# voidful/DeSTA2.5-Audio

Hardware: AMD Instinct MI355X
Metric: train steps/sec (node) Whisper-v3+Llama3.1-8B Q-Former6L at 1/2/4/8 MI355X (higher is better)
Workload: dtype bf16

## Files before the change

desta2.5-audio_amd/csrc/gemm_bf16.hip:

```cpp
#include "common.h"
#include "desta_hip.h"
#include <math.h>

#ifndef GEMM_GROUP_M
#define GEMM_GROUP_M 8
#endif

namespace {

typedef __attribute__((ext_vector_type(4))) unsigned u32x4;
typedef __attribute__((ext_vector_type(2))) float f32x2;

constexpr int BM = 128, BN = 128, BK = 64;
constexpr int TILE_BYTES = BM * BK * 2;

struct GemmArgs {
    const bf16_t* A; const bf16_t* B; void* C;
    int M, N, K;
    long lda, ldb, ldc;
    long sA, sB, sC;
    const float* bias;
    const void* res; long ldr; long sR; int res_f32;
    int act;
    int out_f32;
    bf16_t* preact; long ldp; long sP;
    float alpha;
    bf16_t* aux; long lda_x;
    unsigned drop_thresh, seed_lo, seed_hi; float drop_scale;
    int tilesM, tilesN;
    int full_tiles, split;
    union {
        float* ws;
        const float* b_scale;
    };
    int* tickets;
    const float* rms_w; float rms_eps;
    const float* rope_cs; const int* rope_pos; int rope_cols, rope_hd;
    int tail_skip;
};

__device__ __forceinline__ void rope4(const GemmArgs& p, int m, int n0, float (&v)[4]) {
    if (p.rope_cs && n0 < p.rope_cols) {
        const int pos = p.rope_pos[m];
        const float4 cs = *(const float4*)(p.rope_cs + ((long)pos * (p.rope_hd >> 1) + ((n0 & (p.rope_hd - 1)) >> 1)) * 2);
        const float a0 = v[0], b0 = v[1], a1 = v[2], b1 = v[3];
        v[0] = a0 * cs.x - b0 * cs.y; v[1] = b0 * cs.x + a0 * cs.y;
        v[2] = a1 * cs.z - b1 * cs.w; v[3] = b1 * cs.z + a1 * cs.w;
    }
}

__device__ __forceinline__ void gelu4_bf16(float (&v)[4]) {
#pragma unroll
    for (int e = 0; e < 4; ++e) v[e] = gelu_erf_fast(v[e]);
}

__device__ __forceinline__ void glds16(const void* g, void* l) {
    __builtin_amdgcn_global_load_lds((const __attribute__((address_space(1))) void*)g,
                                     (__attribute__((address_space(3))) void*)l, 16, 0, 0);
}

template <bool ROPE = false>
__device__ __forceinline__ void epilogue4(const GemmArgs& p, int z, int m, int n0, const f32x4& a) {
    float v[4];
#pragma unroll
    for (int e = 0; e < 4; ++e) v[e] = a[e] * p.alpha;
    if (p.bias) {
        const float4 b = *(const float4*)(p.bias + n0);
        v[0] += b.x; v[1] += b.y; v[2] += b.z; v[3] += b.w;
    }
    if constexpr (ROPE) rope4(p, m, n0, v);
    if (p.preact) {
        u16x4 o;
#pragma unroll
        for (int e = 0; e < 4; ++e) o[e] = f2bf(v[e]);
        *(u16x4*)(p.preact + (long)z * p.sP + (long)m * p.ldp + n0) = o;
    }
    if (p.act == 1) {
        if (p.out_f32) {
#pragma unroll
            for (int e = 0; e < 4; ++e) v[e] = gelu_erf(v[e]);
        } else {
            gelu4_bf16(v);
        }
    }
    if (p.drop_thresh) {
        const unsigned long base = ((unsigned long)z * p.M + m) * p.N + n0;
#pragma unroll
        for (int e = 0; e < 4; ++e) v[e] = desta_keep(p.seed_lo, p.seed_hi, base + e, p.drop_thresh) ? v[e] * p.drop_scale : 0.f;
    }
    if (p.res) {
        if (p.res_f32) {
            const float4 r = *(const float4*)((const float*)p.res + (long)z * p.sR + (long)m * p.ldr + n0);
            v[0] += r.x; v[1] += r.y; v[2] += r.z; v[3] += r.w;
        } else {
            const u16x4 r = *(const u16x4*)((const bf16_t*)p.res + (long)z * p.sR + (long)m * p.ldr + n0);
#pragma unroll
            for (int e = 0; e < 4; ++e) v[e] += bf2f(r[e]);
        }
    }
    if (p.out_f32) {
        *(float4*)((float*)p.C + (long)z * p.sC + (long)m * p.ldc + n0) = make_float4(v[0], v[1], v[2], v[3]);
    } else {
        u16x4 o;
#pragma unroll
        for (int e = 0; e < 4; ++e) o[e] = f2bf(v[e]);
        *(u16x4*)((bf16_t*)p.C + (long)z * p.sC + (long)m * p.ldc + n0) = o;
    }
}

__device__ __forceinline__ void epilogue4_f32_stream(const GemmArgs& p, int z, int m, int n0, const f32x4& a) {
    const float4 b = *(const float4*)(p.bias + n0);
    const float4 r = *(const float4*)((const float*)p.res + (long)z * p.sR + (long)m * p.ldr + n0);
    *(float4*)((float*)p.C + (long)z * p.sC + (long)m * p.ldc + n0) =
        make_float4((a[0] * p.alpha + b.x) + r.x, (a[1] * p.alpha + b.y) + r.y, (a[2] * p.alpha + b.z) + r.z, (a[3] * p.alpha + b.w) + r.w);
}

template <int MODE = -1>
__device__ __forceinline__ void epilogue_pair_bf16(const GemmArgs& p, int z, int m, bool row_ok, int ncol0, int fq,
                                                   const f32x4& a0, const f32x4& a1) {
    constexpr bool DYN = MODE < 0;
    const bool has_bias = DYN ? p.bias != nullptr : (MODE & 1) != 0;
    const bool has_gelu = DYN ? p.act == 1 : (MODE & 2) != 0;
    const bool has_rope = DYN ? true : (MODE & 4) != 0;
    const bool has_res = DYN ? p.res != nullptr : (MODE & 8) != 0;
    const bool has_pre = DYN ? p.preact != nullptr : (MODE & 16) != 0;
    if (has_res && !p.res_f32 && (p.ldr & 7) == 0 && (p.sR & 7) == 0) {
        float v[2][4];
#pragma unroll
        for (int t = 0; t < 2; ++t) {
            const f32x4& a = t ? a1 : a0;
            const int n0 = ncol0 + t * 16 + fq * 4;
#pragma unroll
            for (int e = 0; e < 4; ++e) v[t][e] = a[e] * p.alpha;
            if (has_bias) {
                const float4 b = *(const float4*)(p.bias + n0);
                v[t][0] += b.x; v[t][1] += b.y; v[t][2] += b.z; v[t][3] += b.w;
            }
            if (has_gelu) gelu4_bf16(v[t]);
        }
        const int col = ncol0 + (fq & 1) * 16 + (fq >> 1) * 8;
        const u16x8 r = *(const u16x8*)((const bf16_t*)p.res + (long)z * p.sR + (long)m * p.ldr + col);
        float w[8];
#pragma unroll
        for (int e = 0; e < 4; ++e) {
            const auto sw = __builtin_amdgcn_permlane16_swap(__float_as_uint(v[0][e]), __float_as_uint(v[1][e]), false, false);
            w[e] = __uint_as_float(sw[0]);
            w[4 + e] = __uint_as_float(sw[1]);
        }
        u16x8 o;
#pragma unroll
        for (int e = 0; e < 8; ++e) o[e] = f2bf(w[e] + bf2f(r[e]));
        if (row_ok) *(u16x8*)((bf16_t*)p.C + (long)z * p.sC + (long)m * p.ldc + col) = o;
        return;
    }
    unsigned pk[2][2];
#pragma unroll
    for (int t = 0; t < 2; ++t) {
        const f32x4& a = t ? a1 : a0;
        const int n0 = ncol0 + t * 16 + fq * 4;
        float v[4];
#pragma unroll
        for (int e = 0; e < 4; ++e) v[e] = a[e] * p.alpha;
        if (has_bias) {
            const float4 b = *(const float4*)(p.bias + n0);
            v[0] += b.x; v[1] += b.y; v[2] += b.z; v[3] += b.w;
        }
        if (has_rope) rope4(p, min(m, p.M - 1), n0, v);
        if (has_gelu) gelu4_bf16(v);
        if (has_res) {
            if (p.res_f32) {
                const float4 r = *(const float4*)((const float*)p.res + (long)z * p.sR + (long)m * p.ldr + n0);
                v[0] += r.x; v[1] += r.y; v[2] += r.z; v[3] += r.w;
            } else {
                const u16x4 r = *(const u16x4*)((const bf16_t*)p.res + (long)z * p.sR + (long)m * p.ldr + n0);
#pragma unroll
                for (int e = 0; e < 4; ++e) v[e] += bf2f(r[e]);
            }
        }
        pk[t][0] = (unsigned)f2bf(v[0]) | ((unsigned)f2bf(v[1]) << 16);
        pk[t][1] = (unsigned)f2bf(v[2]) | ((unsigned)f2bf(v[3]) << 16);
    }
    const auto lo = __builtin_amdgcn_permlane16_swap(pk[0][0], pk[1][0], false, false);
    const auto hi = __builtin_amdgcn_permlane16_swap(pk[0][1], pk[1][1], false, false);
    const int col = ncol0 + (fq & 1) * 16 + (fq >> 1) * 8;
    if (row_ok) {
        const uint4 o = make_uint4(lo[0], hi[0], lo[1], hi[1]);
        *(uint4*)((bf16_t*)p.C + (long)z * p.sC + (long)m * p.ldc + col) = o;
        if (has_pre) *(uint4*)(p.preact + (long)z * p.sP + (long)m * p.ldp + col) = o;
    }
}

__device__ __forceinline__ uint4 pair_swap_pk(unsigned x0, unsigned x1, unsigned y0, unsigned y1) {
    const auto lo = __builtin_amdgcn_permlane16_swap(x0, y0, false, false);
    const auto hi = __builtin_amdgcn_permlane16_swap(x1, y1, false, false);
    return make_uint4(lo[0], hi[0], lo[1], hi[1]);
}
__device__ __forceinline__ unsigned pk2(float a, float b) { return (unsigned)f2bf(a) | ((unsigned)f2bf(b) << 16); }

__device__ __forceinline__ void epilogue_swiglu_fwd(const GemmArgs& p, int z, int m, bool row_ok, int ncol0, int fq,
                                                    const f32x4& a0, const f32x4& a1, const f32x4& a2, const f32x4& a3) {
    float g[2][4], u[2][4], o[2][4];
#pragma unroll
    for (int e = 0; e < 4; ++e) {
        g[0][e] = bf2f(f2bf(a0[e] * p.alpha)); g[1][e] = bf2f(f2bf(a1[e] * p.alpha));
        u[0][e] = bf2f(f2bf(a2[e] * p.alpha)); u[1][e] = bf2f(f2bf(a3[e] * p.alpha));
    }
#pragma unroll
    for (int t = 0; t < 2; ++t)
#pragma unroll
        for (int e = 0; e < 4; ++e) {
            const float sg = g[t][e] / (1.0f + __expf(-g[t][e]));
            o[t][e] = bf2f(f2bf(sg)) * u[t][e];
        }
    const int col8 = (fq & 1) * 16 + (fq >> 1) * 8;
    const uint4 vg = pair_swap_pk(pk2(g[0][0], g[0][1]), pk2(g[0][2], g[0][3]), pk2(g[1][0], g[1][1]), pk2(g[1][2], g[1][3]));
    const uint4 vu = pair_swap_pk(pk2(u[0][0], u[0][1]), pk2(u[0][2], u[0][3]), pk2(u[1][0], u[1][1]), pk2(u[1][2], u[1][3]));
    const uint4 vo = pair_swap_pk(pk2(o[0][0], o[0][1]), pk2(o[0][2], o[0][3]), pk2(o[1][0], o[1][1]), pk2(o[1][2], o[1][3]));
    if (row_ok) {
        bf16_t* c = (bf16_t*)p.C + (long)z * p.sC + (long)m * p.ldc + ncol0 + col8;
        *(uint4*)c = vg;
        *(uint4*)(c + 32) = vu;
        *(uint4*)(p.aux + (long)m * p.lda_x + (ncol0 >> 1) + col8) = vo;
    }
}
__device__ __forceinline__ void epilogue_swiglu_bwd(const GemmArgs& p, int z, int m, bool row_ok, int ncol0, int fq,
                                                    const f32x4& a0, const f32x4& a1, const f32x4& a2, const f32x4& a3) {
    const int col8 = (fq & 1) * 16 + (fq >> 1) * 8;
#pragma unroll
    for (int h = 0; h < 2; ++h) {
        const f32x4& x = h ? a2 : a0;
        const f32x4& y = h ? a3 : a1;
        float d[8];
#pragma unroll
        for (int e = 0; e < 4; ++e) {
            const auto sw = __builtin_amdgcn_permlane16_swap(__float_as_uint(bf2f(f2bf(x[e] * p.alpha))), __float_as_uint(bf2f(f2bf(y[e] * p.alpha))), false, false);
            d[e] = __uint_as_float(sw[0]);
            d[4 + e] = __uint_as_float(sw[1]);
        }
        const long off = (long)m * p.lda_x + 2 * (ncol0 + 32 * h) + col8;
        const u16x8 gv = *(const u16x8*)(p.aux + off);
        const u16x8 uv = *(const u16x8*)(p.aux + off + 32);
        u16x8 og, ou;
#pragma unroll
        for (int e = 0; e < 8; ++e) {
            const float gg = bf2f(gv[e]), uu = bf2f(uv[e]);
            const float sig = 1.0f / (1.0f + __expf(-gg));
            const float sg = gg * sig;
            ou[e] = f2bf(d[e] * sg);
            og[e] = f2bf(d[e] * uu * (sig * (1.0f + gg * (1.0f - sig))));
        }
        if (row_ok) {
            bf16_t* c = (bf16_t*)p.C + (long)z * p.sC + (long)m * p.ldc + 2 * (ncol0 + 32 * h) + col8;
            *(u16x8*)c = og;
            *(u16x8*)(c + 32) = ou;
        }
    }
}

__device__ __forceinline__ int tr_swz(int k) { return (k & 3) | (((k >> 3) & 3) << 2); }
__device__ __forceinline__ bf16x8 frag_trans(const char* img, int out0, int kk, int fr, int fq) {
    typedef __attribute__((ext_vector_type(4))) __bf16 bf16x4_t;
    const int col = out0 + 4 * (fr & 3);
    bf16x8 o;
#pragma unroll
    for (int s2 = 0; s2 < 2; ++s2) {
        const int k = kk * 32 + 8 * fq + 4 * s2 + (fr >> 2);
        const int off = k * 256 + (((col >> 3) ^ tr_swz(k)) << 4) + ((col & 4) << 1);
        const bf16x4_t v = __builtin_amdgcn_ds_read_tr16_b64_v4bf16((__attribute__((address_space(3))) bf16x4_t*)(img + off));
        o[4 * s2 + 0] = v[0]; o[4 * s2 + 1] = v[1]; o[4 * s2 + 2] = v[2]; o[4 * s2 + 3] = v[3];
    }
    return o;
}

template <bool TA, bool TB>
__global__ __launch_bounds__(256, 2) void gemm_bf16_nt_kernel(GemmArgs p) {
    __shared__ __attribute__((aligned(16))) char lds[2 * 2 * TILE_BYTES];

    const int tid = threadIdx.x, lane = tid & 63, wave = tid >> 6;
    const int wr = wave >> 1, wc = wave & 1;

    const int ntile = p.tilesM * p.tilesN;
    const int L = xcd_remap(blockIdx.x, ntile);
    constexpr int GROUP_M = 8;
    const int gspan = GROUP_M * p.tilesN;
    const int first_m = (L / gspan) * GROUP_M;
    const int gsz = min(p.tilesM - first_m, GROUP_M);
    const int tm = first_m + (L % gspan) % gsz;
    const int tn = (L % gspan) / gsz;
    const int brow = tm * BM, bcol = tn * BN;
    const int z = blockIdx.y;

    const bf16_t* A = p.A + (long)z * p.sA;
    const bf16_t* B = p.B + (long)z * p.sB;

    const bf16_t* srcA[4];
    const bf16_t* srcB[4];
#pragma unroll
    for (int i = 0; i < 4; ++i) {
        const int idx = i * 256 + tid;
        if (TA) {
            const int k = idx >> 4, c = (idx & 15) ^ tr_swz(k);
            srcA[i] = A + (long)k * p.lda + min(brow + c * 8, p.M - 8);
        } else {
            const int r = idx >> 3, c = (idx & 7) ^ (r & 7);
            srcA[i] = A + (long)min(brow + r, p.M - 1) * p.lda + c * 8;
        }
        if (TB) {
            const int k = idx >> 4, c = (idx & 15) ^ tr_swz(k);
            srcB[i] = B + (long)k * p.ldb + min(bcol + c * 8, p.N - 8);
        } else {
// ... 351 lines not shown
#define KTILE_2PHASE(STAGE, WAIT)                                                                              \
    {                                                                                                          \
        _Pragma("unroll") for (int i = 0; i < 2; ++i)                                                          \
            _Pragma("unroll") for (int kk = 0; kk < 2; ++kk) {                                                 \
                b0[i][kk] = *(const bf16x8*)(B0 + (offB[i] ^ (kk << 6)));                                      \
                b1[i][kk] = *(const bf16x8*)(B1 + (offB[i] ^ (kk << 6)));                                      \
            }                                                                                                  \
        _Pragma("unroll") for (int i = 0; i < 4; ++i)                                                          \
            _Pragma("unroll") for (int kk = 0; kk < 2; ++kk) a[i][kk] = *(const bf16x8*)(A0 + (offA[i] ^ (kk << 6))); \
        st.STAGE(g + 7);                                                                                       \
        asm volatile("s_waitcnt lgkmcnt(0)" ::: "memory");                                                     \
        if (STAGGER) { st.WAIT(g + 8); __builtin_amdgcn_s_barrier(); }                                         \
        MFMA_SLOT(0, 0, b0)                                                                                    \
        MFMA_SLOT(0, 2, b1)                                                                                    \
        st.WAIT(g + 8); __builtin_amdgcn_s_barrier();                                                          \
        _Pragma("unroll") for (int i = 0; i < 4; ++i)                                                          \
            _Pragma("unroll") for (int kk = 0; kk < 2; ++kk) a[i][kk] = *(const bf16x8*)(A1 + (offA[i] ^ (kk << 6))); \
        st.STAGE(g + 8);                                                                                       \
        st.STAGE(g + 9);                                                                                       \
        st.STAGE(g + 10);                                                                                      \
        asm volatile("s_waitcnt lgkmcnt(0)" ::: "memory");                                                     \
        if (STAGGER) { st.WAIT(g + 11); __builtin_amdgcn_s_barrier(); }                                       \
        MFMA_SLOT(4, 2, b1)                                                                                    \
        MFMA_SLOT(4, 0, b0)                                                                                    \
        st.WAIT(g + 11); __builtin_amdgcn_s_barrier();                                                         \
    }
    if (STAGGER && wave >= 4) __builtin_amdgcn_s_barrier();
    const int nk_steady = max(nk - 2, 0);
    for (int t = 0; t < nk_steady; ++t) {
        const char* base = lds + (t & 1) * 4 * HT;
        const char* A0 = base, *A1 = base + HT, *B0 = base + 2 * HT, *B1 = base + 3 * HT;
        const int g = 4 * t;
        KTILE_2PHASE(stage_steady, wait_steady)
    }
    at_tail();
    for (int t = nk_steady; t < nk; ++t) {
        const char* base = lds + (t & 1) * 4 * HT;
        const char* A0 = base, *A1 = base + HT, *B0 = base + 2 * HT, *B1 = base + 3 * HT;
        const int g = 4 * t;
        KTILE_2PHASE(stage, tail_wait)
    }
    if (STAGGER && wave < 4) __builtin_amdgcn_s_barrier();
#undef KTILE_2PHASE
#undef MFMA_SLOT
}

constexpr int E256_DYN = -2, E256_SWIGLU_FWD = 32, E256_SWIGLU_BWD = 33, E256_F32_STREAM = 64;
template <int EPI>
__device__ __forceinline__ void k256_epilogue(const GemmArgs& p, int z, int brow, int bcol, int wm, int wn, int fr, int fq,
                                              const f32x4 (&acc)[8][4]) {
    if constexpr (EPI == E256_SWIGLU_FWD || EPI == E256_SWIGLU_BWD) {
        const int ncol0 = bcol + wn * 64;
        if (ncol0 < p.N) {
#pragma unroll
            for (int i = 0; i < 8; ++i) {
                const int m = brow + wm * 128 + i * 16 + fr;
                if (EPI == E256_SWIGLU_FWD) epilogue_swiglu_fwd(p, z, min(m, p.M - 1), m < p.M, ncol0, fq, acc[i][0], acc[i][1], acc[i][2], acc[i][3]);
                else epilogue_swiglu_bwd(p, z, min(m, p.M - 1), m < p.M, ncol0, fq, acc[i][0], acc[i][1], acc[i][2], acc[i][3]);
            }
        }
        return;
    }
#define DESTA_WIDE_TILE(MODE)                                                                                          \
        _Pragma("unroll") for (int i = 0; i < 8; ++i) {                                                                \
            const int m = brow + wm * 128 + i * 16 + fr;                                                               \
            const int mc = min(m, p.M - 1);                                                                            \
            _Pragma("unroll") for (int j = 0; j < 4; j += 2) {                                                         \
                const int ncol0 = bcol + wn * 64 + j * 16;                                                             \
                if (ncol0 >= p.N) continue;                                                          \
                epilogue_pair_bf16<MODE>(p, z, mc, m < p.M, ncol0, fq, acc[i][j], acc[i][j + 1]);    \
            }                                                                                                          \
        }
#define DESTA_F32_STREAM_TILE()                                                                                        \
        _Pragma("unroll") for (int i = 0; i < 8; ++i) {                                                                \
            const int m = brow + wm * 128 + i * 16 + fr;                                                               \
            if (m >= p.M) continue;                                                                                    \
            _Pragma("unroll") for (int j = 0; j < 4; ++j) {                                                            \
                const int n0 = bcol + wn * 64 + j * 16 + fq * 4;                                                       \
                if (n0 >= p.N) continue;                                                                               \
                epilogue4_f32_stream(p, z, m, n0, acc[i][j]);                                                          \
            }                                                                                                          \
        }
    if constexpr (EPI == E256_F32_STREAM) {
        DESTA_F32_STREAM_TILE()
    } else if constexpr (EPI >= 0) {
        DESTA_WIDE_TILE(EPI)
    } else {
        const bool pre_ok = !p.preact || (p.act == 0 && !p.res && (p.ldp & 7) == 0 && (p.sP & 7) == 0);
        const bool wide = !p.out_f32 && pre_ok && p.act <= 1 && !p.drop_thresh && (p.N % 32 == 0) && (p.ldc % 8 == 0);
        if (wide) {
            DESTA_WIDE_TILE(-1)
            return;
        }
#pragma unroll
        for (int i = 0; i < 8; ++i) {
            const int m = brow + wm * 128 + i * 16 + fr;
            if (m >= p.M) continue;
#pragma unroll
            for (int j = 0; j < 4; ++j) {
                const int n0 = bcol + wn * 64 + j * 16 + fq * 4;
                if (n0 >= p.N) continue;
                epilogue4(p, z, m, n0, acc[i][j]);
            }
        }
    }
#undef DESTA_F32_STREAM_TILE
#undef DESTA_WIDE_TILE
}

__device__ __forceinline__ void k256_store_slab(float* slab, int wm, int wn, int fr, int fq, const f32x4 (&acc)[8][4]) {
#pragma unroll
    for (int i = 0; i < 8; ++i)
#pragma unroll
        for (int j = 0; j < 4; ++j)
            *(f32x4*)(slab + (wm * 128 + i * 16 + fr) * 256 + wn * 64 + j * 16 + fq * 4) = acc[i][j];
}

template <bool STAGGER, int PHASES, int EPI = 0>
__global__ __launch_bounds__(512, 2) void gemm_bf16_nt_256_kernel(GemmArgs p) {
    __shared__ __attribute__((aligned(16))) char lds[2 * 4 * HT];

    const int tid = threadIdx.x, lane = tid & 63, wave = __builtin_amdgcn_readfirstlane(tid >> 6);
    const int wm = wave >> 2, wn = wave & 3;

    int L, slice = 0;
    if ((int)blockIdx.x < p.full_tiles) {
        L = xcd_remap(blockIdx.x, p.full_tiles);
    } else {
        const int j = blockIdx.x - p.full_tiles;
        L = p.full_tiles + j / p.split;
        slice = j % p.split;
    }
    constexpr int GROUP_M = GEMM_GROUP_M;
    const int gspan = GROUP_M * p.tilesN;
    const int first_m = (L / gspan) * GROUP_M;
    const int gsz = min(p.tilesM - first_m, GROUP_M);
    const int tm = first_m + (L % gspan) % gsz;
    const int tn = (L % gspan) / gsz;
    const int brow = tm * 256, bcol = tn * 256;
    const int z = blockIdx.y;
    const bf16_t* A = p.A + (long)z * p.sA;
    const bf16_t* B = p.B + (long)z * p.sB;

    const int nk_all = p.K / BK;
    const bool partial = (int)blockIdx.x >= p.full_tiles && p.split > 1;
    const int kt0 = partial ? (int)((long)nk_all * slice / p.split) : 0;
    const int kt1 = partial ? (int)((long)nk_all * (slice + 1) / p.split) : nk_all;
    const int nk = kt1 - kt0;
    K256Stream st;
    st.init(p, lds, tid, wave, A, B, brow, bcol, kt0, nk, PHASES == 2 && p.tail_skip != 0);

    f32x4 acc[8][4];
#pragma unroll
    for (int i = 0; i < 8; ++i)
#pragma unroll
        for (int j = 0; j < 4; ++j) acc[i][j] = f32x4{0.f, 0.f, 0.f, 0.f};

    const int fr = lane & 15, fq = lane >> 4;
    int offA[4], offB[2];
// ... 79 lines not shown
    asm volatile("s_waitcnt vmcnt(0)" ::: "memory");

    if (partial) {
        float* slab = p.ws + ((long)z * (p.tilesM * p.tilesN - p.full_tiles) * p.split +
                              (long)(blockIdx.x - p.full_tiles)) * (256 * 256);
        k256_store_slab(slab, wm, wn, fr, fq, acc);
        if (!p.tickets) return;
        __shared__ int s_go;
        int* tk = p.tickets + 2 * ((long)z * (p.tilesM * p.tilesN - p.full_tiles) + (L - p.full_tiles));
        asm volatile("s_waitcnt vmcnt(0)" ::: "memory");
        __syncthreads();
        if (tid == 0) {
            __builtin_amdgcn_fence(__ATOMIC_RELEASE, "agent");
            asm volatile("s_waitcnt vmcnt(0)" ::: "memory");
            __hip_atomic_fetch_add(tk, 1, __ATOMIC_RELAXED, __HIP_MEMORY_SCOPE_AGENT);
            int spins = 0, ok = 1;
            while (__hip_atomic_load(tk, __ATOMIC_RELAXED, __HIP_MEMORY_SCOPE_AGENT) < p.split) {
                __builtin_amdgcn_s_sleep(2);
                if (++spins > (1 << 21)) { ok = 0; break; }
            }
            __builtin_amdgcn_fence(__ATOMIC_ACQUIRE, "agent");
            asm volatile("s_waitcnt vmcnt(0)" ::: "memory");
            s_go = ok;
        }
        __syncthreads();
        if (s_go) {
            const float* s0 = p.ws + ((long)z * (p.tilesM * p.tilesN - p.full_tiles) + (L - p.full_tiles)) * p.split * (256 * 256);
            const int r0 = 256 * slice / p.split, r1 = 256 * (slice + 1) / p.split;
            for (int idx = tid; idx < (r1 - r0) * 64; idx += 512) {
                const int ml = r0 + (idx >> 6), nl = (idx & 63) * 4;
                const float* q = s0 + ml * 256 + nl;
                f32x4 v = *(const f32x4*)q;
                for (int s2 = 1; s2 < p.split; ++s2) {
                    const f32x4 w = *(const f32x4*)(q + (long)s2 * (256 * 256));
                    v[0] += w[0]; v[1] += w[1]; v[2] += w[2]; v[3] += w[3];
                }
                const int m = brow + ml, n0 = bcol + nl;
                if (m < p.M && n0 < p.N) epilogue4<true>(p, z, m, n0, v);
            }
        }
        __syncthreads();
        if (tid == 0) {
            const int dpt = __hip_atomic_fetch_add(tk + 1, 1, __ATOMIC_RELAXED, __HIP_MEMORY_SCOPE_AGENT);
            if (dpt == p.split - 1) {
                __hip_atomic_store(tk, 0, __ATOMIC_RELAXED, __HIP_MEMORY_SCOPE_AGENT);
                __hip_atomic_store(tk + 1, 0, __ATOMIC_RELAXED, __HIP_MEMORY_SCOPE_AGENT);
            }
        }
        return;
    }
    if constexpr (EPI == 1) {
        const int ncol0 = bcol + wn * 64;
        if (ncol0 < p.N) {
#pragma unroll
            for (int i = 0; i < 8; ++i) {
                const int m = brow + wm * 128 + i * 16 + fr;
                if (p.act == 2) epilogue_swiglu_fwd(p, z, min(m, p.M - 1), m < p.M, ncol0, fq, acc[i][0], acc[i][1], acc[i][2], acc[i][3]);
                else epilogue_swiglu_bwd(p, z, min(m, p.M - 1), m < p.M, ncol0, fq, acc[i][0], acc[i][1], acc[i][2], acc[i][3]);
            }
        }
        return;
    }
    const bool pre_ok = !p.preact || (p.act == 0 && !p.res && (p.ldp & 7) == 0 && (p.sP & 7) == 0);
    const bool wide = !p.out_f32 && pre_ok && p.act <= 1 && !p.drop_thresh && (p.N % 32 == 0) && (p.ldc % 8 == 0);
    if (wide) {
#define DESTA_WIDE_TILE(MODE)                                                                                          \
        _Pragma("unroll") for (int i = 0; i < 8; ++i) {                                                                \
            const int m = brow + wm * 128 + i * 16 + fr;                                                               \
            const int mc = min(m, p.M - 1);                                                                            \
            _Pragma("unroll") for (int j = 0; j < 4; j += 2) {                                                         \
                const int ncol0 = bcol + wn * 64 + j * 16;                                                             \
                if (ncol0 >= p.N) continue;                                                          \
                epilogue_pair_bf16<MODE>(p, z, mc, m < p.M, ncol0, fq, acc[i][j], acc[i][j + 1]);    \
            }                                                                                                          \
        }
        const int mode = (p.bias ? 1 : 0) | (p.act == 1 ? 2 : 0) | (p.rope_cs ? 4 : 0) | (p.res ? 8 : 0) | (p.preact ? 16 : 0);
        if (mode == 0) { DESTA_WIDE_TILE(0) }
        else if (mode == 8) { DESTA_WIDE_TILE(8) }
        else if (mode == 4) { DESTA_WIDE_TILE(4) }
        else if (mode == 1) { DESTA_WIDE_TILE(1) }
        else if (mode == 3) { DESTA_WIDE_TILE(3) }
        else if (mode == 16) { DESTA_WIDE_TILE(16) }
        else { DESTA_WIDE_TILE(-1) }
#undef DESTA_WIDE_TILE
        return;
    }
    if (p.out_f32 && p.bias && p.res && p.res_f32 && !p.preact && p.act == 0 && !p.drop_thresh) {
#pragma unroll
        for (int i = 0; i < 8; ++i) {
            const int m = brow + wm * 128 + i * 16 + fr;
            if (m >= p.M) continue;
#pragma unroll
            for (int j = 0; j < 4; ++j) {
                const int n0 = bcol + wn * 64 + j * 16 + fq * 4;
                if (n0 >= p.N) continue;
                epilogue4_f32_stream(p, z, m, n0, acc[i][j]);
            }
        }
        return;
    }
#pragma unroll
    for (int i = 0; i < 8; ++i) {
        const int m = brow + wm * 128 + i * 16 + fr;
        if (m >= p.M) continue;
#pragma unroll
        for (int j = 0; j < 4; ++j) {
            const int n0 = bcol + wn * 64 + j * 16 + fq * 4;
            if (n0 >= p.N) continue;
            epilogue4(p, z, m, n0, acc[i][j]);
        }
    }
}

template <int EPI>
__global__ __launch_bounds__(512, 2) void gemm_bf16_nt_256p_kernel(GemmArgs p, int* queue) {
    __shared__ __attribute__((aligned(16))) char lds[2 * 4 * HT + 16];
    int* s_ticket = (int*)(lds + 2 * 4 * HT);
    const int tid = threadIdx.x, lane = tid & 63, wave = __builtin_amdgcn_readfirstlane(tid >> 6);
    const int wm = wave >> 2, wn = wave & 3;
    const int fr = lane & 15, fq = lane >> 4;
    constexpr int GROUP_M = GEMM_GROUP_M;
    const int nk_all = p.K / BK;

    const int xq = blockIdx.x & 7;
    const int F = p.full_tiles, q8 = F >> 3, r8 = F & 7;
    const int lo = (xq < r8) ? xq * (q8 + 1) : r8 * (q8 + 1) + (xq - r8) * q8;
    const int n_full = q8 + (xq < r8 ? 1 : 0);
    const int n_split_items = p.split > 1 ? (p.tilesM * p.tilesN - F) * p.split : 0;
    const int n_items = n_full + (n_split_items > xq ? (n_split_items - xq + 7) >> 3 : 0);
    int* counter = queue + xq;

    int brow, bcol, kt0, nk, slab;
    bool partial;
    auto geometry = [&](int tk) {
        int L, slice = 0;
        partial = tk >= n_full;
        if (!partial) {
            L = lo + tk;
        } else {
            slab = xq + 8 * (tk - n_full);
            L = F + slab / p.split;
            slice = slab % p.split;
        }
        const int gspan = GROUP_M * p.tilesN;
        const int first_m = (L / gspan) * GROUP_M;
        const int gsz = min(p.tilesM - first_m, GROUP_M);
        brow = (first_m + (L % gspan) % gsz) * 256;
        bcol = ((L % gspan) / gsz) * 256;
        kt0 = partial ? (int)((long)nk_all * slice / p.split) : 0;
        const int kt1 = partial ? (int)((long)nk_all * (slice + 1) / p.split) : nk_all;
        nk = kt1 - kt0;
// ... 503 lines not shown
        g_skinny = value;
    }
    else if (option == 4) g_phases2 = value;
    else if (option == 5) g_inkernel_splitk = value;
    else if (option == 6) g_small_ring = value;
    else if (option == 10) g_tail_skip = value;
    else if (option == 11) {
        if (value != 0 && value != 162 && value != 164) { desta_set_error("gemm_set_option: FP8 skinny variant %d unknown (162 164)", value); return DESTA_EINVAL; }
        g_skinny_w8 = value;
    }
    else if (option == 3) {
        if (value < 1 || value > 65535) { desta_set_error("gemm_set_option: skinny grid %d out of range", value); return DESTA_EINVAL; }
        g_skinny_blocks = value;
    }
    else { desta_set_error("gemm_set_option: unknown option %d", option); return DESTA_EINVAL; }
    return DESTA_OK;
}

extern "C" int desta_gemm_bf16_nt(const desta_gemm_desc* d, void* stream) {
    DESTA_CHECK_ARG(d && d->A && d->B && d->C, "gemm: null operand");
    DESTA_CHECK_ARG(d->M > 0 && d->N > 0 && d->K > 0, "gemm: bad shape M=%d N=%d K=%d", d->M, d->N, d->K);
    DESTA_CHECK_ARG(d->K % BK == 0, "gemm: K=%d must be a multiple of %d", d->K, BK);
    DESTA_CHECK_ARG(d->N % 4 == 0, "gemm: N=%d must be a multiple of 4", d->N);
    DESTA_CHECK_ARG(d->lda % 8 == 0 && d->ldb % 8 == 0 && d->ldc % 4 == 0, "gemm: lda/ldb must be multiples of 8, ldc of 4");
    DESTA_CHECK_ARG(((uintptr_t)d->A % 16 == 0) && ((uintptr_t)d->B % 16 == 0) && ((uintptr_t)d->C % 16 == 0),
                    "gemm: operands must be 16-byte aligned");
    DESTA_CHECK_ARG(d->batch >= 1 && d->batch <= 65535, "gemm: bad batch %d", d->batch);
    DESTA_CHECK_ARG(!d->residual || d->ldr % 4 == 0, "gemm: ldr must be a multiple of 4");
    DESTA_CHECK_ARG(!d->preact || d->ldp % 4 == 0, "gemm: ldp must be a multiple of 4");
    DESTA_CHECK_ARG(!d->trans_a || (d->M % 8 == 0 && d->M >= 8), "gemm: trans_a needs M to be a multiple of 8");
    DESTA_CHECK_ARG(!d->trans_b || (d->N % 8 == 0 && d->N >= 8), "gemm: trans_b needs N to be a multiple of 8");
    DESTA_CHECK_ARG(!(d->trans_a || d->trans_b) || (d->act != 4 && !d->a_rms_weight), "gemm: trans_a / trans_b not available on the decode path");
    GemmArgs a;
    a.A = (const bf16_t*)d->A; a.B = (const bf16_t*)d->B; a.C = d->C;
    a.M = d->M; a.N = d->N; a.K = d->K;
    a.lda = d->lda; a.ldb = d->ldb; a.ldc = d->ldc;
    a.sA = d->stride_a; a.sB = d->stride_b; a.sC = d->stride_c;
    a.bias = d->bias;
    a.res = d->residual; a.ldr = d->ldr; a.sR = d->stride_r; a.res_f32 = d->residual_f32;
    a.act = d->act; a.out_f32 = d->out_f32; a.tail_skip = g_tail_skip;
    a.preact = (bf16_t*)d->preact; a.ldp = d->ldp; a.sP = d->stride_p;
    a.alpha = d->alpha;
    a.aux = (bf16_t*)d->aux; a.lda_x = d->ld_aux;
    DESTA_CHECK_ARG(d->dropout_p >= 0.f && d->dropout_p < 1.f, "gemm: dropout_p must be in [0,1)");
    a.drop_thresh = d->dropout_p > 0.f ? desta_drop_thresh(d->dropout_p) : 0u;
    a.drop_scale = 1.0f / (1.0f - d->dropout_p);
    a.seed_lo = (unsigned)d->dropout_seed; a.seed_hi = (unsigned)(d->dropout_seed >> 32);
    DESTA_CHECK_ARG(d->act >= 0 && d->act <= 4, "gemm: unknown act %d", d->act);
    DESTA_CHECK_ARG(d->act < 2 || d->act == 4 || (d->aux && !d->out_f32 && !d->bias && !d->residual && !d->preact && d->ld_aux % 8 == 0),
                    "gemm: SwiGLU epilogues need aux, bf16 output and no bias/residual/preact");
    DESTA_CHECK_ARG(d->act != 3 || d->ldc % 8 == 0, "gemm: act 3 needs ldc (2N-wide rows) to be a multiple of 8");
    DESTA_CHECK_ARG((d->act != 2 && d->act != 3) || (d->N % 64 == 0 && d->ldc % 8 == 0 && d->batch == 1 && !d->trans_a && !d->trans_b && d->dropout_p == 0.f),
                    "gemm: the SwiGLU epilogues work on whole 64-column blocks (N %% 64 == 0), row-major operands, batch 1");
    constexpr int NCU = 256;
    const int tM = (d->M + 255) / 256, tN = (d->N + 255) / 256, nk = d->K / BK;
    const long T = (long)tM * tN;
    int split = 1, full = (int)T;
    if (d->batch == 1 && d->workspace && nk >= 8 && d->act != 2 && d->act != 3) {
        const int rem = (int)(T % NCU);
        if (rem > 0 && rem <= NCU / 2) {
            int sp = NCU / rem;
            if (sp > 8) sp = 8;
            if (sp > nk / 16) sp = nk / 16;
            if (sp >= 2 && (size_t)rem * sp * 256 * 256 * sizeof(float) + 4096 <= d->workspace_bytes) { split = sp; full = (int)(T - rem); }
        }
    }
    a.rope_cs = d->rope_cos_sin; a.rope_pos = d->rope_pos; a.rope_cols = d->rope_cols; a.rope_hd = d->rope_head_dim;
    if (d->rope_cos_sin)
        DESTA_CHECK_ARG(d->rope_pos && (d->rope_head_dim == 64 || d->rope_head_dim == 128) && d->rope_cols > 0 && d->rope_cols <= d->N &&
                        d->rope_cols % d->rope_head_dim == 0 && d->act == 0 && !d->bias && !d->residual && !d->preact && !d->out_f32 &&
                        d->dropout_p == 0.f && d->batch == 1 && d->M > 16 && !d->trans_a && !d->trans_b && d->N % 32 == 0 && d->ldc % 8 == 0,
                        "gemm: the rotary epilogue needs rope_pos, head_dim 64 / 128, rope_cols a multiple of it, a plain bf16 output (no bias / residual / act) and M > 16");
    a.rms_w = d->a_rms_weight; a.rms_eps = d->a_rms_eps;
    if (d->a_rms_weight)
        DESTA_CHECK_ARG(d->M <= 16 && (size_t)d->M * 2 * (size_t)d->K <= (size_t)SKINNY_XS_BYTES && d->K % 512 == 0 &&
                        (d->act == 0 || d->act == 4) && g_force_variant == 0,
                        "gemm: a_rms_weight (fused RMSNorm of A) needs M <= 16, M*2K <= %d bytes of LDS, K %% 512 == 0, act 0 or 4", SKINNY_XS_BYTES);
    if (d->act == 4 || (d->M <= 16 && g_force_variant == 0 && !d->trans_a && !d->trans_b && d->act != 2 && d->act != 3)) {
        DESTA_CHECK_ARG(d->act != 4 || (d->M <= 16 && !d->out_f32 && !d->bias && !d->residual && !d->preact && d->dropout_p == 0.f),
                        "gemm: act 4 (SwiGLU over concatenated gate|up rows) is the decode path: M <= 16, bf16 out, no other epilogue");
        int cols = 16, u = 2;
        if (g_skinny && d->act != 4) { cols = g_skinny / 10; u = g_skinny % 10; }
        const int ntiles = d->act == 4 ? (d->N + 7) / 8 : (d->N + cols - 1) / cols;
        a.tilesM = 1; a.tilesN = ntiles; a.full_tiles = ntiles; a.split = 1; a.ws = nullptr; a.tickets = nullptr;
        const dim3 grid(ntiles < g_skinny_blocks ? ntiles : g_skinny_blocks, d->batch);
        hipStream_t st = (hipStream_t)stream;
        const bool rms = a.rms_w != nullptr;
#define SK_LAUNCH(C_, U_, SW_) \
        do { if (rms) hipLaunchKernelGGL((gemm_bf16_nt_skinny_kernel<C_, U_, SW_, true>), grid, dim3(512), 0, st, a, ntiles); \
             else hipLaunchKernelGGL((gemm_bf16_nt_skinny_kernel<C_, U_, SW_, false>), grid, dim3(512), 0, st, a, ntiles); } while (0)
        if (d->act == 4) SK_LAUNCH(16, 2, true);
        else if (cols == 64) SK_LAUNCH(64, 1, false);
        else if (cols == 32) SK_LAUNCH(32, 2, false);
        else if (u == 4) SK_LAUNCH(16, 4, false);
        else SK_LAUNCH(16, 2, false);
#undef SK_LAUNCH
        DESTA_CHECK_LAUNCH("gemm_bf16_nt_skinny");
        g_last_kernel = 3;
        return DESTA_OK;
    }
    bool big = false;
    if (d->M >= 128 && d->N >= 128 && d->K >= 512) {
        const double rounds = (double)full * d->batch / NCU + (split > 1 ? 1.0 / split : 0.0);
        const double ideal = (double)T * d->batch / NCU;
        const double eff = ideal / (split > 1 ? rounds : ceil(rounds));
        big = eff >= 0.78;
// ... 327 lines not shown
```

Measured before the change: 6.603.

## Batch epilogue global loads ahead of compute in 256-tile GEMM epilogues

Restructures the 256x256 GEMM epilogues (SwiGLU backward, bias/GELU/rotary pair epilogues, f32 residual stream) so the bias, rope cos/sin, aux gate/up and residual loads for several row groups are issued together before the arithmetic. Scheduling barriers and empty asm markers fence the pieces. The aim is to hide global-load latency that previously sat serialized inside each row's epilogue. It also adds a host-side aliasing check between C and the residual/bias/aux/rope inputs, which the early loads make necessary. The cost is higher register pressure at 2 waves per SIMD and fragile compiler-scheduling hints.

New measurement: 6.647, median of 6. Within noise of the previous version (+0.7%).

```diff
diff --git a/desta2.5-audio_amd/csrc/gemm_bf16.hip b/desta2.5-audio_amd/csrc/gemm_bf16.hip
--- a/desta2.5-audio_amd/csrc/gemm_bf16.hip
+++ b/desta2.5-audio_amd/csrc/gemm_bf16.hip
@@ -48,6 +48,18 @@
         v[2] = a1 * cs.z - b1 * cs.w; v[3] = b1 * cs.z + a1 * cs.w;
     }
 }
+__device__ __forceinline__ void rope4_cs(const GemmArgs& p, int n0, const float4& cs, float (&v)[4]) {
+    if (n0 < p.rope_cols) {
+        const float a0 = v[0], b0 = v[1], a1 = v[2], b1 = v[3];
+        float a0x = a0 * cs.x, b0y = b0 * cs.y;
+        const float b0x = b0 * cs.x, b1w = b1 * cs.w, a1w = a1 * cs.w;
+        asm("" : "+v"(a0x), "+v"(b0y));
+        v[0] = a0x - b0y;
+        v[1] = __builtin_fmaf(a0, cs.y, b0x);
+        v[2] = __builtin_fmaf(a1, cs.z, -b1w);
+        v[3] = __builtin_fmaf(b1, cs.z, a1w);
+    }
+}
 
 __device__ __forceinline__ void gelu4_bf16(float (&v)[4]) {
 #pragma unroll
@@ -108,16 +120,29 @@
     }
 }
 
-__device__ __forceinline__ void epilogue4_f32_stream(const GemmArgs& p, int z, int m, int n0, const f32x4& a) {
-    const float4 b = *(const float4*)(p.bias + n0);
-    const float4 r = *(const float4*)((const float*)p.res + (long)z * p.sR + (long)m * p.ldr + n0);
+__device__ __forceinline__ void epilogue4_f32_stream_finish(const GemmArgs& p, int z, int m, int n0, const f32x4& a, const float4& b, const float4& r) {
     *(float4*)((float*)p.C + (long)z * p.sC + (long)m * p.ldc + n0) =
         make_float4((a[0] * p.alpha + b.x) + r.x, (a[1] * p.alpha + b.y) + r.y, (a[2] * p.alpha + b.z) + r.z, (a[3] * p.alpha + b.w) + r.w);
 }
 
-template <int MODE = -1>
+struct PairOps { f32x4 bias[2]; f32x4 cs[2]; };
+template <class V> __device__ __forceinline__ void landed(V& v) { asm volatile("" : "+v"(v)); }
+__device__ __forceinline__ float4 as_float4(const f32x4& v) { return make_float4(v[0], v[1], v[2], v[3]); }
+__device__ __forceinline__ int pair_rope_pos(const GemmArgs& p, int m) { return p.rope_pos[m]; }
+__device__ __forceinline__ void pair_load_bias(const GemmArgs& p, int ncol0, int fq, PairOps& o) {
+#pragma unroll
+    for (int t = 0; t < 2; ++t) o.bias[t] = *(const f32x4*)(p.bias + ncol0 + t * 16 + fq * 4);
+}
+__device__ __forceinline__ void pair_load_cs(const GemmArgs& p, int pos, int ncol0, int fq, PairOps& o) {
+#pragma unroll
+    for (int t = 0; t < 2; ++t) {
+        const int n0 = ncol0 + t * 16 + fq * 4;
+        o.cs[t] = *(const f32x4*)(p.rope_cs + ((long)pos * (p.rope_hd >> 1) + ((n0 & (p.rope_hd - 1)) >> 1)) * 2);
+    }
+}
+template <int MODE = -1, bool PRE = false>
 __device__ __forceinline__ void epilogue_pair_bf16(const GemmArgs& p, int z, int m, bool row_ok, int ncol0, int fq,
-                                                   const f32x4& a0, const f32x4& a1) {
+                                                   const f32x4& a0, const f32x4& a1, const PairOps* ops = nullptr) {
     constexpr bool DYN = MODE < 0;
     const bool has_bias = DYN ? p.bias != nullptr : (MODE & 1) != 0;
     const bool has_gelu = DYN ? p.act == 1 : (MODE & 2) != 0;
@@ -133,7 +158,7 @@
 #pragma unroll
             for (int e = 0; e < 4; ++e) v[t][e] = a[e] * p.alpha;
             if (has_bias) {
-                const float4 b = *(const float4*)(p.bias + n0);
+                const float4 b = PRE ? as_float4(ops->bias[t]) : *(const float4*)(p.bias + n0);
                 v[t][0] += b.x; v[t][1] += b.y; v[t][2] += b.z; v[t][3] += b.w;
             }
             if (has_gelu) gelu4_bf16(v[t]);
@@ -162,10 +187,13 @@
 #pragma unroll
         for (int e = 0; e < 4; ++e) v[e] = a[e] * p.alpha;
         if (has_bias) {
-            const float4 b = *(const float4*)(p.bias + n0);
+            const float4 b = PRE ? as_float4(ops->bias[t]) : *(const float4*)(p.bias + n0);
             v[0] += b.x; v[1] += b.y; v[2] += b.z; v[3] += b.w;
         }
-        if (has_rope) rope4(p, min(m, p.M - 1), n0, v);
+        if (has_rope) {
+            if constexpr (PRE) rope4_cs(p, n0, as_float4(ops->cs[t]), v);
+            else rope4(p, min(m, p.M - 1), n0, v);
+        }
         if (has_gelu) gelu4_bf16(v);
         if (has_res) {
             if (p.res_f32) {
@@ -223,8 +251,17 @@
         *(uint4*)(p.aux + (long)m * p.lda_x + (ncol0 >> 1) + col8) = vo;
     }
 }
-__device__ __forceinline__ void epilogue_swiglu_bwd(const GemmArgs& p, int z, int m, bool row_ok, int ncol0, int fq,
-                                                    const f32x4& a0, const f32x4& a1, const f32x4& a2, const f32x4& a3) {
+__device__ __forceinline__ void epilogue_swiglu_bwd_load(const GemmArgs& p, int m, int ncol0, int fq, u16x8 (&gu)[4]) {
+    const int col8 = (fq & 1) * 16 + (fq >> 1) * 8;
+#pragma unroll
+    for (int h = 0; h < 2; ++h) {
+        const long off = (long)m * p.lda_x + 2 * (ncol0 + 32 * h) + col8;
+        gu[2 * h] = *(const u16x8*)(p.aux + off);
+        gu[2 * h + 1] = *(const u16x8*)(p.aux + off + 32);
+    }
+}
+__device__ __forceinline__ void epilogue_swiglu_bwd_finish(const GemmArgs& p, int z, int m, bool row_ok, int ncol0, int fq,
+                                                           const f32x4& a0, const f32x4& a1, const f32x4& a2, const f32x4& a3, const u16x8 (&gu)[4]) {
     const int col8 = (fq & 1) * 16 + (fq >> 1) * 8;
 #pragma unroll
     for (int h = 0; h < 2; ++h) {
@@ -237,9 +274,7 @@
             d[e] = __uint_as_float(sw[0]);
             d[4 + e] = __uint_as_float(sw[1]);
         }
-        const long off = (long)m * p.lda_x + 2 * (ncol0 + 32 * h) + col8;
-        const u16x8 gv = *(const u16x8*)(p.aux + off);
-        const u16x8 uv = *(const u16x8*)(p.aux + off + 32);
+        const u16x8 gv = gu[2 * h], uv = gu[2 * h + 1];
         u16x8 og, ou;
 #pragma unroll
         for (int e = 0; e < 8; ++e) {
@@ -256,6 +291,145 @@
         }
     }
 }
+__device__ __forceinline__ void epilogue_swiglu_bwd(const GemmArgs& p, int z, int m, bool row_ok, int ncol0, int fq,
+                                                    const f32x4& a0, const f32x4& a1, const f32x4& a2, const f32x4& a3) {
+    u16x8 gu[4];
+    epilogue_swiglu_bwd_load(p, m, ncol0, fq, gu);
+    epilogue_swiglu_bwd_finish(p, z, m, row_ok, ncol0, fq, a0, a1, a2, a3, gu);
+}
+
+__device__ __forceinline__ void k256_epilogue_waits_counted() { __builtin_amdgcn_s_waitcnt(0xC07F); }
+#ifndef E256_RG_ACT3
+#define E256_RG_ACT3 4
+#endif
+#ifndef E256_RG_ROPE
+#define E256_RG_ROPE 2
+#endif
+#ifndef E256_RG_F32
+#define E256_RG_F32 2
+#endif
+#define K256_PIECE_FENCE() __builtin_amdgcn_sched_barrier(0)
+__device__ __forceinline__ void k256_swiglu_bwd_tile(const GemmArgs& p, int z, int brow, int ncol0, int wm, int fr, int fq,
+                                                     const f32x4 (&acc)[8][4]) {
+    k256_epilogue_waits_counted();
+#pragma unroll
+    for (int i0 = 0; i0 < 8; i0 += E256_RG_ACT3) {
+        u16x8 gu[E256_RG_ACT3][4];
+#pragma unroll
+        for (int ii = 0; ii < E256_RG_ACT3; ++ii) {
+            K256_PIECE_FENCE();
+            epilogue_swiglu_bwd_load(p, min(brow + wm * 128 + (i0 + ii) * 16 + fr, p.M - 1), ncol0, fq, gu[ii]);
+        }
+#pragma unroll
+        for (int ii = 0; ii < E256_RG_ACT3; ++ii) {
+            const int i = i0 + ii, m = brow + wm * 128 + i * 16 + fr;
+            K256_PIECE_FENCE();
+#pragma unroll
+            for (int q = 0; q < 4; ++q) landed(gu[ii][q]);
+            epilogue_swiglu_bwd_finish(p, z, min(m, p.M - 1), m < p.M, ncol0, fq, acc[i][0], acc[i][1], acc[i][2], acc[i][3], gu[ii]);
+        }
+        K256_PIECE_FENCE();
+    }
+}
+
+template <int MODE>
+__device__ __forceinline__ void k256_wide_tile_loaded(const GemmArgs& p, int z, int brow, int bcol, int wm, int wn, int fr, int fq,
+                                                      const f32x4 (&acc)[8][4]) {
+    constexpr bool BIAS = (MODE & 1) != 0, ROPE = (MODE & 4) != 0;
+    static_assert(MODE > 0 && (MODE & ~7) == 0 && (BIAS || ROPE), "bias / bias + GELU / rotary");
+    constexpr int RG = ROPE ? E256_RG_ROPE : 8;
+    const int col0 = bcol + wn * 64;
+    const int lcol[2] = {min(col0, p.N - 32), min(col0 + 32, p.N - 32)};
+    k256_epilogue_waits_counted();
+    PairOps cb[2];
+    int pos[8];
+    if constexpr (BIAS) {
+#pragma unroll
+        for (int jj = 0; jj < 2; ++jj) pair_load_bias(p, lcol[jj], fq, cb[jj]);
+    }
+    if constexpr (ROPE) {
+#pragma unroll
+        for (int i = 0; i < 8; ++i) pos[i] = pair_rope_pos(p, min(brow + wm * 128 + i * 16 + fr, p.M - 1));
+    }
+#pragma unroll
+    for (int i0 = 0; i0 < 8; i0 += RG) {
+        PairOps ops[RG][2];
+        K256_PIECE_FENCE();
+        if constexpr (ROPE) {
+#pragma unroll
+            for (int ii = 0; ii < RG; ++ii) {
+                K256_PIECE_FENCE();
+#pragma unroll
+                for (int jj = 0; jj < 2; ++jj) pair_load_cs(p, pos[i0 + ii], lcol[jj], fq, ops[ii][jj]);
+            }
+        }
+        if constexpr (BIAS) {
+            if (i0 == 0) {
+                K256_PIECE_FENCE();
+#pragma unroll
+                for (int jj = 0; jj < 2; ++jj) { landed(cb[jj].bias[0]); landed(cb[jj].bias[1]); }
+            }
+        }
+#pragma unroll
+        for (int ii = 0; ii < RG; ++ii) {
+            const int i = i0 + ii, m = brow + wm * 128 + i * 16 + fr;
+#pragma unroll
+            for (int jj = 0; jj < 2; ++jj) {
+                const int ncol0 = col0 + jj * 32;
+                if constexpr (ROPE) {
+                    K256_PIECE_FENCE();
+                    landed(ops[ii][jj].cs[0]); landed(ops[ii][jj].cs[1]);
+                }
+                if (ncol0 >= p.N) continue;
+                if constexpr (BIAS) { ops[ii][jj].bias[0] = cb[jj].bias[0]; ops[ii][jj].bias[1] = cb[jj].bias[1]; }
+                epilogue_pair_bf16<MODE, true>(p, z, min(m, p.M - 1), m < p.M, ncol0, fq, acc[i][2 * jj], acc[i][2 * jj + 1], &ops[ii][jj]);
+            }
+        }
+    }
+    K256_PIECE_FENCE();
+}
+
+__device__ __forceinline__ void k256_f32_stream_tile(const GemmArgs& p, int z, int brow, int bcol, int wm, int wn, int fr, int fq,
+                                                     const f32x4 (&acc)[8][4]) {
+    f32x4 b[4];
+    int nc[4];
+    k256_epilogue_waits_counted();
+#pragma unroll
+    for (int j = 0; j < 4; ++j) {
+        nc[j] = min(bcol + wn * 64 + j * 16 + fq * 4, p.N - 4);
+        b[j] = *(const f32x4*)(p.bias + nc[j]);
+    }
+#pragma unroll
+    for (int i0 = 0; i0 < 8; i0 += E256_RG_F32) {
+        f32x4 r[E256_RG_F32][4];
+        K256_PIECE_FENCE();
+#pragma unroll
+        for (int ii = 0; ii < E256_RG_F32; ++ii) {
+            const int mc = min(brow + wm * 128 + (i0 + ii) * 16 + fr, p.M - 1);
+            K256_PIECE_FENCE();
+#pragma unroll
+            for (int j = 0; j < 4; ++j) r[ii][j] = *(const f32x4*)((const float*)p.res + (long)z * p.sR + (long)mc * p.ldr + nc[j]);
+        }
+        if (i0 == 0) {
+            K256_PIECE_FENCE();
+#pragma unroll
+            for (int j = 0; j < 4; ++j) landed(b[j]);
+        }
+#pragma unroll
+        for (int ii = 0; ii < E256_RG_F32; ++ii) {
+            const int i = i0 + ii, m = brow + wm * 128 + i * 16 + fr;
+#pragma unroll
+            for (int j = 0; j < 4; ++j) {
+                const int n0 = bcol + wn * 64 + j * 16 + fq * 4;
+                K256_PIECE_FENCE();
+                landed(r[ii][j]);
+                if (m < p.M && n0 < p.N) epilogue4_f32_stream_finish(p, z, m, n0, acc[i][j], as_float4(b[j]), as_float4(r[ii][j]));
+            }
+        }
+    }
+    K256_PIECE_FENCE();
+}
+#undef K256_PIECE_FENCE
 
 __device__ __forceinline__ int tr_swz(int k) { return (k & 3) | (((k >> 3) & 3) << 2); }
 __device__ __forceinline__ bf16x8 frag_trans(const char* img, int out0, int kk, int fr, int fq) {
@@ -713,11 +887,14 @@
     if constexpr (EPI == E256_SWIGLU_FWD || EPI == E256_SWIGLU_BWD) {
         const int ncol0 = bcol + wn * 64;
         if (ncol0 < p.N) {
-#pragma unroll
-            for (int i = 0; i < 8; ++i) {
-                const int m = brow + wm * 128 + i * 16 + fr;
-                if (EPI == E256_SWIGLU_FWD) epilogue_swiglu_fwd(p, z, min(m, p.M - 1), m < p.M, ncol0, fq, acc[i][0], acc[i][1], acc[i][2], acc[i][3]);
-                else epilogue_swiglu_bwd(p, z, min(m, p.M - 1), m < p.M, ncol0, fq, acc[i][0], acc[i][1], acc[i][2], acc[i][3]);
+            if constexpr (EPI == E256_SWIGLU_BWD) {
+                k256_swiglu_bwd_tile(p, z, brow, ncol0, wm, fr, fq, acc);
+            } else {
+#pragma unroll
+                for (int i = 0; i < 8; ++i) {
+                    const int m = brow + wm * 128 + i * 16 + fr;
+                    epilogue_swiglu_fwd(p, z, min(m, p.M - 1), m < p.M, ncol0, fq, acc[i][0], acc[i][1], acc[i][2], acc[i][3]);
+                }
             }
         }
         return;
@@ -732,18 +909,10 @@
                 epilogue_pair_bf16<MODE>(p, z, mc, m < p.M, ncol0, fq, acc[i][j], acc[i][j + 1]);    \
             }                                                                                                          \
         }
-#define DESTA_F32_STREAM_TILE()                                                                                        \
-        _Pragma("unroll") for (int i = 0; i < 8; ++i) {                                                                \
-            const int m = brow + wm * 128 + i * 16 + fr;                                                               \
-            if (m >= p.M) continue;                                                                                    \
-            _Pragma("unroll") for (int j = 0; j < 4; ++j) {                                                            \
-                const int n0 = bcol + wn * 64 + j * 16 + fq * 4;                                                       \
-                if (n0 >= p.N) continue;                                                                               \
-                epilogue4_f32_stream(p, z, m, n0, acc[i][j]);                                                          \
-            }                                                                                                          \
-        }
     if constexpr (EPI == E256_F32_STREAM) {
-        DESTA_F32_STREAM_TILE()
+        k256_f32_stream_tile(p, z, brow, bcol, wm, wn, fr, fq, acc);
+    } else if constexpr (EPI == 1 || EPI == 3 || EPI == 4) {
+        k256_wide_tile_loaded<EPI>(p, z, brow, bcol, wm, wn, fr, fq, acc);
     } else if constexpr (EPI >= 0) {
         DESTA_WIDE_TILE(EPI)
     } else {
@@ -765,7 +934,6 @@
             }
         }
     }
-#undef DESTA_F32_STREAM_TILE
 #undef DESTA_WIDE_TILE
 }
 
@@ -951,11 +1119,14 @@
     if constexpr (EPI == 1) {
         const int ncol0 = bcol + wn * 64;
         if (ncol0 < p.N) {
-#pragma unroll
-            for (int i = 0; i < 8; ++i) {
-                const int m = brow + wm * 128 + i * 16 + fr;
-                if (p.act == 2) epilogue_swiglu_fwd(p, z, min(m, p.M - 1), m < p.M, ncol0, fq, acc[i][0], acc[i][1], acc[i][2], acc[i][3]);
-                else epilogue_swiglu_bwd(p, z, min(m, p.M - 1), m < p.M, ncol0, fq, acc[i][0], acc[i][1], acc[i][2], acc[i][3]);
+            if (p.act == 2) {
+#pragma unroll
+                for (int i = 0; i < 8; ++i) {
+                    const int m = brow + wm * 128 + i * 16 + fr;
+                    epilogue_swiglu_fwd(p, z, min(m, p.M - 1), m < p.M, ncol0, fq, acc[i][0], acc[i][1], acc[i][2], acc[i][3]);
+                }
+            } else {
+                k256_swiglu_bwd_tile(p, z, brow, ncol0, wm, fr, fq, acc);
             }
         }
         return;
@@ -976,26 +1147,16 @@
         const int mode = (p.bias ? 1 : 0) | (p.act == 1 ? 2 : 0) | (p.rope_cs ? 4 : 0) | (p.res ? 8 : 0) | (p.preact ? 16 : 0);
         if (mode == 0) { DESTA_WIDE_TILE(0) }
         else if (mode == 8) { DESTA_WIDE_TILE(8) }
-        else if (mode == 4) { DESTA_WIDE_TILE(4) }
-        else if (mode == 1) { DESTA_WIDE_TILE(1) }
-        else if (mode == 3) { DESTA_WIDE_TILE(3) }
+        else if (mode == 4) k256_wide_tile_loaded<4>(p, z, brow, bcol, wm, wn, fr, fq, acc);
+        else if (mode == 1) k256_wide_tile_loaded<1>(p, z, brow, bcol, wm, wn, fr, fq, acc);
+        else if (mode == 3) k256_wide_tile_loaded<3>(p, z, brow, bcol, wm, wn, fr, fq, acc);
         else if (mode == 16) { DESTA_WIDE_TILE(16) }
         else { DESTA_WIDE_TILE(-1) }
 #undef DESTA_WIDE_TILE
         return;
     }
     if (p.out_f32 && p.bias && p.res && p.res_f32 && !p.preact && p.act == 0 && !p.drop_thresh) {
-#pragma unroll
-        for (int i = 0; i < 8; ++i) {
-            const int m = brow + wm * 128 + i * 16 + fr;
-            if (m >= p.M) continue;
-#pragma unroll
-            for (int j = 0; j < 4; ++j) {
-                const int n0 = bcol + wn * 64 + j * 16 + fq * 4;
-                if (n0 >= p.N) continue;
-                epilogue4_f32_stream(p, z, m, n0, acc[i][j]);
-            }
-        }
+        k256_f32_stream_tile(p, z, brow, bcol, wm, wn, fr, fq, acc);
         return;
     }
 #pragma unroll
@@ -1605,6 +1766,21 @@
     DESTA_CHECK_ARG(d->act != 3 || d->ldc % 8 == 0, "gemm: act 3 needs ldc (2N-wide rows) to be a multiple of 8");
     DESTA_CHECK_ARG((d->act != 2 && d->act != 3) || (d->N % 64 == 0 && d->ldc % 8 == 0 && d->batch == 1 && !d->trans_a && !d->trans_b && d->dropout_p == 0.f),
                     "gemm: the SwiGLU epilogues work on whole 64-column blocks (N %% 64 == 0), row-major operands, batch 1");
+    {
+        const size_t c_es = d->out_f32 ? 4 : 2;
+        const char* c0 = (const char*)d->C;
+        const char* c1 = c0 + ((size_t)(d->batch - 1) * (size_t)d->stride_c + (size_t)(d->M - 1) * (size_t)d->ldc + (size_t)(d->act == 3 ? 2 * d->N : d->N)) * c_es;
+        auto overlaps = [&](const void* q, size_t bytes) { return q && (const char*)q < c1 && (const char*)q + bytes > c0; };
+        if (d->residual) {
+            const size_t r_es = d->residual_f32 ? 4 : 2;
+            const bool in_place = d->residual == d->C && r_es == c_es && d->ldr == d->ldc && (d->batch == 1 || d->stride_r == d->stride_c);
+            DESTA_CHECK_ARG(in_place || !overlaps(d->residual, ((size_t)(d->batch - 1) * (size_t)d->stride_r + (size_t)(d->M - 1) * (size_t)d->ldr + (size_t)d->N) * r_es),
+                            "gemm: C overlaps the residual without being the in-place update (same address, type and strides)");
+        }
+        DESTA_CHECK_ARG(!overlaps(d->bias, (size_t)d->N * 4), "gemm: C overlaps the bias");
+        DESTA_CHECK_ARG(d->act != 3 || !overlaps(d->aux, ((size_t)(d->M - 1) * (size_t)d->ld_aux + 2 * (size_t)d->N) * 2), "gemm: act 3: C overlaps the saved gate|up (aux)");
+        DESTA_CHECK_ARG(!d->rope_cos_sin || !overlaps(d->rope_pos, (size_t)d->M * 4), "gemm: C overlaps rope_pos");
+    }
     constexpr int NCU = 256;
     const int tM = (d->M + 255) / 256, tN = (d->N + 255) / 256, nk = d->K / BK;
     const long T = (long)tM * tN;
```
